# zoltanmaric/h264-fer

Measured on AMD Instinct MI355X. Metric: macroblocks/sec encode (1080p full-search ME) + bit-exact bitstream vs ref, higher is better.
Workload: dtype u8; 1 GPU; 1080p IPPP encode, full-search +-16 ME (BASELINE configs[2]); content=textured, coded_size=1920x1072, streams_per_gpu=256, contexts_per_gpu=1, gop=30, qp=12, window=32, maxdiff=3, parallelism=1 x 256 independent closed-GOP streams

## Files before the change

### h264-fer_amd/csrc/fer_me.hip

```cpp
#include <stdlib.h>
#include "fer_internal.h"
#include "fer_mvpred.h"
#include "fer_chain_idx.h"

#define INF_M 1000000000

struct WList {
    int m;
    int xy;
};

__device__ __forceinline__ int pack_xy(int x, int y) { return (x & 0xffff) | (y << 16); }
__device__ __forceinline__ int unp_x(int xy) { return (int)(short)(xy & 0xffff); }
__device__ __forceinline__ int unp_y(int xy) { return xy >> 16; }

__device__ __forceinline__ void wl_insert(WList &L, int K, int lane, bool valid, int m, int xy)
{
    int thr = lane_bcast(L.m, K - 1);
    unsigned long long mask = __ballot(valid && m < thr);
    while (mask) {
        int src = __ffsll((long long)mask) - 1;
        mask &= mask - 1;
        int cm = lane_bcast(m, src), cxy = lane_bcast(xy, src);
        int pos = __popcll(__ballot(lane < K && L.m <= cm));
        if (pos < K) {
            int um = FER_DPP(L.m, DPP_WAVE_SHR1), uxy = FER_DPP(L.xy, DPP_WAVE_SHR1);
            if (lane > pos && lane < K) {
                L.m = um;
                L.xy = uxy;
            } else if (lane == pos) {
                L.m = cm;
                L.xy = cxy;
            }
        }
    }
}

#define WAVE_LDS_SYNC()                                    \
    do {                                                   \
        __builtin_amdgcn_fence(__ATOMIC_SEQ_CST, "wavefront"); \
        __builtin_amdgcn_wave_barrier();                   \
    } while (0)
__device__ __forceinline__ int lds_rank64(const unsigned *p, unsigned mine, int n4 = 16)
{
    const uint4 *q = (const uint4 *)p;
    int r = 0;
#pragma unroll 4
    for (int i = 0; i < n4; i++) {
        uint4 k = q[i];
        r += (int)(k.x < mine) + (int)(k.y < mine) + (int)(k.z < mine) + (int)(k.w < mine);
    }
    return r;
}

template <int NB, bool ORDERED, class RAW, class FIN, class ARR>
__device__ __forceinline__ bool select_topk_ex(const int (&v)[NB], int K, int lane, int *sel, WList &L, RAW raw, FIN fin, ARR arr)
{
    unsigned *A = (unsigned *)sel, *B = A + 64;
    int *Ci = sel + 128, *Di = sel + 192;
    const unsigned long long lt = (1ull << lane) - 1ull;
    int lmin = 0x7fffffff, lmax = -1, total = 0;
#pragma unroll
    for (int u = 0; u < NB; u++) {
        total += __popcll(__ballot(v[u] >= 0));
        lmin = (int)min((unsigned)lmin, (unsigned)v[u]);
        lmax = max(lmax, v[u]);
    }
    const int need = min(K, total);
    L.m = INF_M;
    L.xy = 0;
    if (need == 0) return true;
    int c = 65;
    if (!__any(lmax >= (1 << 26))) {
        B[lane] = 0xffffffffu;
        int T0 = 0x7fffffff;
        if (__popcll(__ballot(lmin != 0x7fffffff)) >= need) {
            int lo = 0, hi = (1 << 21) - 1;
            if (__popcll(__ballot(lmin <= hi)) >= need) {
                while (lo < hi) {
                    const int mid = (lo + hi) >> 1;
                    if (__popcll(__ballot(lmin <= mid)) >= need)
                        hi = mid;
                    else
                        lo = mid + 1;
                }
                T0 = lo;
            } else {
                T0 = 1 << 21;
            }
        }
        WAVE_LDS_SYNC();
        if (T0 < (1 << 21) && NB * 64 <= 2048) {
            int nsurv = 0;
#pragma unroll
            for (int u = 0; u < NB; u++) {
                const bool take = (unsigned)v[u] <= (unsigned)T0;
                const unsigned long long mk = __ballot(take);
                if (mk) {
                    const int slot = nsurv + (int)__builtin_amdgcn_mbcnt_hi((uint32_t)(mk >> 32), __builtin_amdgcn_mbcnt_lo((uint32_t)mk, 0u));
                    if (take && slot < 64) {
                        B[slot] = ((unsigned)v[u] << 11) | (unsigned)arr(u);
                        Ci[slot] = raw(u);
                    }
                    nsurv += __popcll(mk);
                }
            }
            WAVE_LDS_SYNC();
            c = nsurv;
        }
    }
    if (c <= 64) {
        WAVE_LDS_SYNC();
        const unsigned mine = B[lane];
        const int mypay = Ci[lane];
        const int rk = lds_rank64(B, mine, (__builtin_amdgcn_readfirstlane(c) + 3) >> 2);
        WAVE_LDS_SYNC();
        if (lane < c && rk < need) {
            A[rk] = mine >> 11;
            Di[rk] = mypay;
        }
        WAVE_LDS_SYNC();
        if (lane < need) {
            L.m = (int)A[lane];
            L.xy = fin(Di[lane]);
        }
        WAVE_LDS_SYNC();
        return true;
    }
    if (!ORDERED) return false;
    int *key = sel, *kxy = sel + 64, *key2 = sel + 128, *kxy2 = sel + 192;
    int lo = wave_min(lmin), hi;
    if (__popcll(__ballot(lmin != 0x7fffffff)) >= need)
        hi = wave_max(lmin != 0x7fffffff ? lmin : -1);
    else
        hi = wave_max(lmax);
    while (lo < hi) {
        int mid = lo + ((hi - lo) >> 1);
        int cnt = 0;
#pragma unroll
        for (int u = 0; u < NB; u++) cnt += __popcll(__ballot(v[u] >= 0 && v[u] <= mid));
        if (cnt >= need)
            hi = mid;
        else
            lo = mid + 1;
    }
    const int T = lo;
    int c_less = 0;
#pragma unroll
    for (int u = 0; u < NB; u++) c_less += __popcll(__ballot(v[u] >= 0 && v[u] < T));
    const int take_eq = need - c_less;
    int nsel = 0, eq_seen = 0;
    WAVE_LDS_SYNC();
#pragma unroll
    for (int u = 0; u < NB; u++) {
        bool ok = v[u] >= 0;
        bool eq = ok && v[u] == T;
        unsigned long long meq = __ballot(eq);
        bool take = (ok && v[u] < T) || (eq && eq_seen + __popcll(meq & lt) < take_eq);
        unsigned long long mt = __ballot(take);
        if (take) {
            int pos = nsel + __popcll(mt & lt);
            key[pos] = v[u];
            kxy[pos] = raw(u);
        }
        nsel += __popcll(mt);
        eq_seen += __popcll(meq);
    }
    WAVE_LDS_SYNC();
    int mk = lane < need ? key[lane] : INF_M, mxy = lane < need ? kxy[lane] : 0;
    int rank = 0;
    for (int i = 0; i < need; i++) {
        int ki = key[i];
        rank += (ki < mk) || (ki == mk && i < lane);
    }
    if (lane < need) {
        key2[rank] = mk;
        kxy2[rank] = mxy;
    }
    WAVE_LDS_SYNC();
    if (lane < need) {
        L.m = key2[lane];
        L.xy = fin(kxy2[lane]);
    }
    WAVE_LDS_SYNC();
    return true;
}
template <int NB, class RAW, class FIN>
__device__ __forceinline__ void select_topk(const int (&v)[NB], int K, int lane, int *sel, WList &L, RAW raw, FIN fin)
{
    select_topk_ex<NB, true>(v, K, lane, sel, L, raw, fin, [&](int u) { return u * 64 + lane; });
}

typedef unsigned short u16x2_t __attribute__((ext_vector_type(2)));
typedef short i16x2_t __attribute__((ext_vector_type(2)));
__device__ __forceinline__ uint32_t pk_sub16(uint32_t a, uint32_t b)
{
    return __builtin_bit_cast(uint32_t, (u16x2_t)(__builtin_bit_cast(u16x2_t, a) - __builtin_bit_cast(u16x2_t, b)));
}
__device__ __forceinline__ uint32_t pk_abs16(uint32_t a)
{
    i16x2_t x = __builtin_bit_cast(i16x2_t, a), z = {0, 0};
    return __builtin_bit_cast(uint32_t, __builtin_elementwise_max(x, (i16x2_t)(z - x)));
}
struct SuPk {
    uint32_t s01, s23, s4;
    uint32_t d01, d23, d4;
    uint32_t s12, s34;
    uint32_t e12, e34;
};
__device__ __forceinline__ SuPk su_pack(const int s[5])
{
    SuPk p;
    p.s01 = (uint32_t)s[0] | ((uint32_t)s[1] << 16);
    p.s23 = (uint32_t)s[2] | ((uint32_t)s[3] << 16);
    p.s4 = (uint32_t)s[4];
    p.d01 = (uint32_t)(s[0] - s[1]) << 16;
    p.d23 = (uint32_t)(s[0] - s[2]) | ((uint32_t)(s[0] - s[3]) << 16);
    p.d4 = (uint32_t)(s[0] - s[4]);
    p.s12 = (uint32_t)s[1] | ((uint32_t)s[2] << 16);
    p.s34 = (uint32_t)s[3] | ((uint32_t)s[4] << 16);
    p.e12 = (uint32_t)(s[0] - s[1]) | ((uint32_t)(s[0] - s[2]) << 16);
    p.e34 = (uint32_t)(s[0] - s[3]) | ((uint32_t)(s[0] - s[4]) << 16);
    return p;
}
__device__ __forceinline__ int feat_dist_w(uint32_t a, uint32_t b, uint32_t c, const SuPk &p)
{
    uint32_t t = __builtin_amdgcn_sad_u16(a, p.s01, 0);
    t = __builtin_amdgcn_sad_u16(b, p.s23, t);
    t = __builtin_amdgcn_sad_u16(c, p.s4, t);
    uint32_t kk = __builtin_amdgcn_perm(a, a, 0x01000100);
    t = __builtin_amdgcn_sad_u16(pk_sub16(kk, a), p.d01, t);
    t = __builtin_amdgcn_sad_u16(pk_sub16(kk, b), p.d23, t);
    t = __builtin_amdgcn_sad_u16(pk_sub16(kk, c) & 0xffffu, p.d4, t);
    return (int)t;
}
__device__ __forceinline__ int feat_dist_rec(const uint16_t *__restrict__ rec, const SuPk &p)
{
    const uint32_t *r = (const uint32_t *)rec;
    return feat_dist_w(r[0], r[1], r[2], p);
}
struct FeatRec {
    uint32_t a, b, c;
};

__device__ __forceinline__ FeatRec feat_rec_direct(const IPlanes &ip, int W, int H, int frac, int refy, int refx)
{
    const int y = iclamp(refy, 0, H - 1), x = iclamp(refx, 0, W - 1);
    const uint8_t *p0 = ip.base + (size_t)frac * ip.plane + (size_t)y * ip.pitch + (x & ~3);
    const uint32_t sh = (uint32_t)(x & 3);
    uint32_t h84[8], hc[8];
#pragma unroll
    for (int r = 0; r < 8; r++) {
        const uint32_t *w = (const uint32_t *)(p0 + (size_t)r * ip.pitch);
        const uint32_t lo = __builtin_amdgcn_alignbyte(w[1], w[0], sh), hi = __builtin_amdgcn_alignbyte(w[2], w[1], sh);
        const uint32_t a4 = __builtin_amdgcn_sad_u8(lo, 0u, 0u);
        h84[r] = __builtin_amdgcn_sad_u8(hi, 0u, a4) | (a4 << 16);
        hc[r] = __builtin_amdgcn_udot4(hi, 0x00000101u, __builtin_amdgcn_udot4(lo, 0x00000101u, 0u, false), false);
    }
    const uint32_t top = h84[0] + h84[1] + h84[2] + h84[3], all = top + h84[4] + h84[5] + h84[6] + h84[7];
    const uint32_t k3 = (h84[0] + h84[1] + h84[4] + h84[5]) & 0xffffu;
    const uint32_t k4 = hc[0] + hc[1] + hc[2] + hc[3] + hc[4] + hc[5] + hc[6] + hc[7];
    FeatRec f;
    f.a = (all & 0xffffu) | (top << 16);
    f.b = (all >> 16) | (k3 << 16);
    f.c = k4;
    return f;
}

template <int R1>
struct LocalGeo {
    static constexpr int N1 = 2 * R1 + 1, PW = 2 * R1 + 8, NC = N1 * N1 * 16, NB = (NC + 63) / 64;
    static constexpr int HTAB = 8 * PW * N1 * 2;
};
template <int R1>
// ... 194 lines not shown
    const unsigned bx = xcd_swizzle(blockIdx.x, gridDim.x);
    const int mb = (int)(bx >> 2), part = (int)(bx & 3);
    const int W = d.W, H = d.H;
    const size_t ysz = d.ysz;
    const uint8_t *Y = d.curY + (size_t)s * ysz;
    const IPlanes ip = ip_stream(d, s);
    const int sx = ((mb % d.mbw) << 4) + (part & 1) * 8, sy = ((mb / d.mbw) << 4) + (part >> 1) * 8;
    const size_t pidx = ((size_t)s * d.nmb + mb) * 4 + part;

#ifdef FER_PROBE
    const bool probe = FER_DBGF(d, 128) && s == 0 && (bx % 997) == 5;
    long long tmark = probe ? wall_clock64() : 0;
#define PP_MARK(k)                                                          \
    if (probe) {                                                            \
        long long now_ = wall_clock64();                                    \
        if (lane == 0) atomicAdd((unsigned long long *)&d.timing[32 + k], (unsigned long long)(now_ - tmark)); \
        tmark = now_;                                                       \
    }
#else
#define PP_MARK(k)
#endif
    constexpr int RRL = (WIN == 16) ? 1 : 2;
    LocalLoads<RRL> ld;
    const bool fast_path = (WIN == 32 || WIN == 16) && !FER_DBGF(d, 3) && !d.basic;
    if (fast_path) local_request<RRL>(ip, W, H, sx - RRL, sy - RRL, lane, ld, 0, 1);
    int px = lane & 7, py = lane >> 3;
    int v = Y[(size_t)(sy + py) * W + sx + px];
    int su[5];
    su[0] = wave_sum(v);
    su[1] = wave_sum(py > 3 ? 0 : v);
    su[2] = wave_sum(px > 3 ? 0 : v);
    su[3] = wave_sum((py & 3) > 1 ? 0 : v);
    su[4] = wave_sum((px & 3) > 1 ? 0 : v);
    if (lane < 5) d.suma[pidx * 5 + lane] = su[lane];
    if (d.basic) {
        if (lane == 0) {
            d.st3n[pidx] = 0;
            d.v0[pidx] = 0;
        }
        return;
    }
    const SuPk sp = su_pack(su);
    PP_MARK(0)

    WList L;
    L.m = INF_M;
    L.xy = 0;
    const int R = window / 2, n = 2 * R + 1;
    const int r2 = window / 16, n2w = 2 * r2 + 1, nloc = n2w * n2w * 16;
    const uint16_t *F0 = d.feat0 + (size_t)s * 6 * ysz;
    const int wb = (n * n + 63) >> 6;
    if ((WIN == 32 || WIN == 16) && !FER_DBGF(d, 3)) {
        constexpr int WCH = 3;
        constexpr int NN = (WIN ? WIN : 32) + 1;
        constexpr int NBc = WIN ? WIN : 32, RPB = 64 / NBc, NWB = (NN + RPB - 1) / RPB;
        constexpr int LB = LocalGeo<RRL>::NB;
        static_assert(LB <= 7, "ME_SEL_NB leaves room for 7 local batches");
        const int ix = lane % NBc, r0 = lane / NBc;
        const int rx = sx - R + ix;
        const bool xok = rx >= 0 && rx < W;
        const int wx = iabs(ix - R) + 4;
        const uint32_t colo = (uint32_t)iclamp(rx, 0, W - 1) * 12u, rowb = (uint32_t)W * 12u;
        auto fin = [&](int idx) {
            if (idx < wb * 64) return pack_xy((idx / n - R) * 4, (idx % n - R) * 4);
            int c = idx - wb * 64;
            int frac = c & 15, pos = c >> 4;
            return pack_xy((pos / n2w - r2) * 4 + (frac & 3), (pos % n2w - r2) * 4 + (frac >> 2));
        };
        uint32_t k0w[NWB];
#pragma unroll
        for (int b2 = 0; b2 < NWB; b2++) {
            const int ry = iclamp(sy - R + b2 * RPB + r0, 0, H - 1);
            k0w[b2] = *(const uint32_t *)((const char *)F0 + (colo + __umul24((uint32_t)ry, rowb)));
        }
        const uint32_t k0c = feat0_load(F0, W, H, sy - R + min(lane, NN - 1), sx + R).a;
        auto second_group = [&](int half) {
            if (half == 0) local_request<RRL>(ip, W, H, sx - RRL, sy - RRL, lane, ld, 1, 2);
        };
        local_metrics<RRL, decltype(second_group), true>(ip, W, H, sx - r2, sy - r2, sp, lane, (uint32_t *)wide_m, sel_lds, 0, 2, &ld, second_group);
        unsigned lminl = 0xffffffffu;
#pragma unroll
        for (int u = 0; u < LB; u++) lminl = min(lminl, (unsigned)sel_lds[u * 64 + lane]);
        int T = 0x7fffffff;
        if (__popcll(__ballot(lminl < (1u << 21))) >= 33) {
            int lo = 0, hi = (1 << 21) - 1;
            while (lo < hi) {
                const int mid = (lo + hi) >> 1;
                if (__popcll(__ballot(lminl <= (unsigned)mid)) >= 33)
                    hi = mid;
                else
                    lo = mid + 1;
            }
            T = lo;
        }
        int *surv = wide_m;
        int ns = 0;
        const uint32_t s0 = (uint32_t)su[0];
        bool done = false;
        if (T != 0x7fffffff) {
            static_assert((NBc / 2) % RPB == 0 && NN <= 64, "a batch stays on one side of the centre row");
            const int iy_lo = max(0, R - sy), iy_hi = min(NN - 1, H - 1 - (sy - R));
            const unsigned long long rowv = ((2ull << iy_hi) - 1ull) & ~((1ull << iy_lo) - 1ull);
            const unsigned long long colv = wave_ballot(xok);
            constexpr unsigned long long GRP = NBc == 64 ? ~0ull : (1ull << NBc) - 1ull;
            const uint32_t w5lo = 5u * (uint32_t)(wx + R - r0), w5hi = 5u * (uint32_t)(wx - R + r0);
            const int arr0 = ix * NN + r0;
#pragma unroll
            for (int b2 = 0; b2 < NWB; b2++) {
                unsigned long long valid = 0;
#pragma unroll
                for (int j = 0; j < RPB; j++)
                    if ((rowv >> (b2 * RPB + j)) & 1ull) valid |= GRP << (j * NBc);
                valid &= colv;
                const uint32_t w5 = b2 * RPB < R ? w5lo - 5u * (uint32_t)(b2 * RPB) : w5hi + 5u * (uint32_t)(b2 * RPB);
                const uint32_t lb = __umul24(w5, __builtin_amdgcn_sad_u16(k0w[b2] & 0xffffu, s0, 0u));
                const unsigned long long mk = wave_ballot(lb <= (uint32_t)T) & valid;
                if (mk) {
                    const int slot = ns + (int)__builtin_amdgcn_mbcnt_hi((uint32_t)(mk >> 32), __builtin_amdgcn_mbcnt_lo((uint32_t)mk, 0u));
                    if (wave_mask_bit(mk) && slot < 128) surv[slot] = arr0 + b2 * RPB;
                    ns += __popcll(mk);
                }
            }
            {
                const uint32_t lb = __umul24(5u * (uint32_t)(R + 4 + iabs(lane - R)), __builtin_amdgcn_sad_u16(k0c & 0xffffu, s0, 0u));
                const unsigned long long mk = sx + R < W ? wave_ballot(lb <= (uint32_t)T) & rowv : 0ull;
                if (mk) {
                    const int slot = ns + (int)__builtin_amdgcn_mbcnt_hi((uint32_t)(mk >> 32), __builtin_amdgcn_mbcnt_lo((uint32_t)mk, 0u));
                    if (wave_mask_bit(mk) && slot < 128) surv[slot] = (NN - 1) * NN + lane;
                    ns += __popcll(mk);
                }
            }
            WAVE_LDS_SYNC();
            if (ns <= 128) {
                int v[2 + LB], ar[2];
#pragma unroll
                for (int b2 = 0; b2 < 2; b2++) {
                    v[b2] = -1;
                    ar[b2] = 0;
                    if (b2 * 64 < ns) {
                        const int idx = b2 * 64 + lane;
                        const bool on = idx < ns;
                        const int ai = on ? surv[idx] : 0;
                        const int cix = ai / NN, ciy = ai - cix * NN;
                        const FeatRec f = feat0_load(F0, W, H, sy - R + ciy, sx - R + cix);
                        const int m = (int)__umul24((uint32_t)(iabs(cix - R) + iabs(ciy - R) + 4), (uint32_t)feat_dist_w(f.a, f.b, f.c, sp));
                        v[b2] = on ? m : -1;
                        ar[b2] = ai;
                    }
                }
#pragma unroll
                for (int u = 0; u < LB; u++) v[2 + u] = sel_lds[u * 64 + lane];
                WAVE_LDS_SYNC();
                auto arrv = [&](int u) { return u < 2 ? ar[u < 2 ? u : 0] : wb * 64 + (u - 2) * 64 + lane; };
                done = select_topk_ex<2 + LB, false>(v, 33, lane, wide_m + 128, L, arrv, fin, arrv);
            }
        }
        PP_MARK(1)
#ifdef FER_STATS
        if (lane == 0) {
            atomicAdd((unsigned long long *)&d.timing[48], 1ull);
            atomicAdd((unsigned long long *)&d.timing[49], done ? 0ull : 1ull);
            atomicAdd((unsigned long long *)&d.timing[50], (unsigned long long)ns);
            atomicAdd((unsigned long long *)&d.timing[51], T == 0x7fffffff ? 1ull : 0ull);
            atomicAdd((unsigned long long *)&d.timing[52], (unsigned long long)(T == 0x7fffffff ? 0 : T));
        }
#endif
        if (!done) {
            WAVE_LDS_SYNC();
            int vloc[LB];
#pragma unroll
            for (int u = 0; u < LB; u++) vloc[u] = sel_lds[u * 64 + lane];
            WAVE_LDS_SYNC();
            auto wide_load = [&](int iy0, FeatRec (&fr)[WCH]) {
#pragma unroll
                for (int q = 0; q < WCH; q++) {
                    int ry = iclamp(sy - R + iy0 + q * RPB + r0, 0, H - 1);
                    const uint32_t *r = (const uint32_t *)((const char *)F0 + (colo + __umul24((uint32_t)ry, rowb)));
                    fr[q].a = r[0];
                    fr[q].b = r[1];
                    fr[q].c = r[2];
                }
            };
            auto wide_eval = [&](int iy0, const FeatRec (&fr)[WCH]) {
#pragma unroll
                for (int q = 0; q < WCH; q++) {
                    const int iy = iy0 + q * RPB + r0;
                    const int ry = sy - R + iy;
                    const int m = (int)__umul24((uint32_t)(wx + iabs(iy - R)), (uint32_t)feat_dist_w(fr[q].a, fr[q].b, fr[q].c, sp));
                    const int bad = (xok && ry >= 0 && ry < H) ? 0 : -1;
                    wide_m[iy < n ? ix * n + iy : ME_WIDE_LDS - 1] = m | bad;
                }
            };
            {
                constexpr int STEP = RPB * WCH;
                FeatRec fa[WCH], fb[WCH];
                wide_load(0, fa);
                for (int iy0 = 0; iy0 < n; iy0 += 2 * STEP) {
                    if (iy0 + STEP < n) wide_load(iy0 + STEP, fb);
                    wide_eval(iy0, fa);
                    if (iy0 + STEP < n) {
                        if (iy0 + 2 * STEP < n) wide_load(iy0 + 2 * STEP, fa);
                        wide_eval(iy0 + STEP, fb);
                    }
                }
            }
            {
                const int iy = min(lane, n - 1);
                const int rxl = sx + R, ry = sy - R + iy;
                FeatRec f = feat0_load(F0, W, H, ry, rxl);
                int m = (R + 4 + iabs(iy - R)) * feat_dist_w(f.a, f.b, f.c, sp);
                if (!(rxl < W && ry >= 0 && ry < H)) m = -1;
                if (lane < n) wide_m[(n - 1) * n + iy] = m;
            }
            __syncthreads();
            int v[ME_SEL_NB];
#pragma unroll
            for (int u = 0; u < ME_SEL_NB; u++) {
                v[u] = -1;
                if (u < wb) {
                    int c = u * 64 + lane;
                    if (c < n * n) v[u] = wide_m[c];
                } else if (u - wb < LB) {
                    v[u] = vloc[u - wb < LB ? u - wb : 0];
                }
            }
            WAVE_LDS_SYNC();
            auto raw = [&](int u) { return u * 64 + lane; };
            PP_MARK(2)
            select_topk<ME_SEL_NB>(v, 33, lane, sel_lds, L, raw, fin);
        }
        PP_MARK(3)
    } else {
        for (int base = 0; base < n * n && !FER_DBGF(d, 1); base += 64) {
            int c = base + lane;
            int tx = c / n - R, ty = c % n - R;
            int rx = sx + tx, ry = sy + ty;
            bool ok = c < n * n && rx >= 0 && rx < W && ry >= 0 && ry < H;
            int m = 0;
            if (ok) m = (iabs(tx) + iabs(ty) + 4) * feat_dist_rec(F0 + ((size_t)ry * W + rx) * 6, sp);
            wl_insert(L, 33, lane, ok, m, pack_xy(tx * 4, ty * 4));
        }
        for (int base = 0; base < nloc && !FER_DBGF(d, 2); base += 64) {
            int c = base + lane;
            int frac = c & 15, pos = c >> 4;
            int tx = pos / n2w - r2, ty = pos % n2w - r2;
            int rx = sx + tx, ry = sy + ty;
            bool ok = c < nloc && rx >= 0 && rx < W && ry >= 0 && ry < H;
            int m = 0;
            if (ok) {
                const FeatRec f = feat_rec_direct(ip, W, H, frac, ry, rx);
                m = (iabs(tx) + iabs(ty) + 4) * feat_dist_w(f.a, f.b, f.c, sp);
            }
            wl_insert(L, 33, lane, ok, m, pack_xy(tx * 4 + (frac & 3), ty * 4 + (frac >> 2)));
        }
    }
    const int n3 = __popcll(__ballot(lane < 33 && L.m < 100000000));
    int v0 = 0;
    if (!FER_DBGF(d, 4)) {
        const SrcBlk SB = src_block_load(Y, W, sx, sy);
        const int cx = unp_x(L.xy), cy = unp_y(L.xy);
        const int sad = sad_lane(ip, W, H, sx, sy, lane < n3 ? cx : 0, lane < n3 ? cy : 0, SB);
        if (lane < n3) {
            int *o = d.st3 + (pidx * 33 + lane) * 3;
            o[0] = cx;
            o[1] = cy;
            o[2] = sad;
        }
        const int wk = wave_min(lane < n3 ? (sad << 6) | lane : 0x7fffffff);
        if (wk != 0x7fffffff) v0 = lane_bcast(L.xy, wk & 63);
    }
    if (lane == 0) {
        d.st3n[pidx] = n3;
        d.v0[pidx] = v0;
    }

}

struct NoProbe {
    __device__ __forceinline__ int operator()(int) const { return 0; }
};
template <bool QUIRK, class SINK, class PROBE = NoProbe>
__device__ __forceinline__ int walk_buckets_q(const FerDev &d, int s, const int (&su)[5], const SuPk &sp, int sx, int sy, int lane,
                                              uint32_t *tbl, int halt_cnt, int &jend, SINK sink, uint32_t max_slice = 0xffffffffu,
                                              bool skip0 = false, PROBE probe = PROBE())
{
    int tren = 0;
    jend = 180;
    const int kt = d.kt;
    const uint32_t *kol2 = d.kol2 + (size_t)s * 16384 * kt;
    const uint32_t *srec = d.sort_rec;
    const int n0 = QUIRK ? d.zero_cnt[s] : 0;
    const uint32_t npos = (uint32_t)(d.W * d.H), g0 = (uint32_t)s * npos;
    const uint16_t *F0 = d.feat0 + (size_t)s * 6 * d.ysz;
    const int t_lo = QUIRK ? 0 : (max(sx - 279, 0) >> d.ktw_shift), t_hi = QUIRK ? kt - 1 : (min(sx + 279, d.W - 1) >> d.ktw_shift);
    auto qstart = [&](int a) -> uint32_t {
        if (a <= 0) return g0;
        if (a == 1) return g0 + min(2u * (uint32_t)n0, npos);
        if (a >= 16384) return g0 + npos;
        return kol2[(size_t)a * kt] - (uint32_t)n0;
    };
    const uint32_t sxy = ((uint32_t)sx << 16) | (uint32_t)sy;
    const char *srec_s = (const char *)(srec + (size_t)g0 * 3);
    auto fetch = [&](unsigned b_start, int b_cnt, uint32_t &r0, uint32_t &r1, uint32_t &r2) {
        const uint32_t li = (b_start - g0) + (unsigned)min(lane, max(b_cnt - 1, 0));
        const uint32_t *e = (const uint32_t *)(srec_s + __umul24(li, 12u));
        r0 = e[0];
        r1 = e[1];
        r2 = e[2];
    };
    auto passes = [&](uint32_t r0, uint32_t r1) -> bool {
        uint32_t dist = __builtin_amdgcn_sad_u16(r0, sxy, 0);
        uint32_t e12 = pk_abs16(pk_sub16(r1, sp.s12));
// ... 385 lines not shown
                };
                if (nout > FER_OUTL) {
                    fallback = true;
                } else {
                    const uint32_t DM = dist_of(m1, m2);
                    const bool members = halves_ok(m1);
                    bigD[q] = members && DM > 0 ? (int)DM : 0x7fffffff;
                    dminN = min(dminN, bigD[q]);
                    const uint32_t *ol = d.boutl + ((size_t)s * d.nlists + (d.kol2[((size_t)s * 16384 + bigA[q]) * d.kt] - g0_) / FER_BRANGE_MIN) * FER_OUTL;
                    for (uint32_t o0 = 0; o0 < nout; o0 += 64) {
                        const bool lv = o0 + (uint32_t)lane < nout;
                        const uint32_t idx = lv ? ol[o0 + lane] : g0_;
                        const uint32_t *rec = d.sort_rec + (size_t)idx * 3;
                        const uint32_t r0 = rec[0], r1 = rec[1], r2 = rec[2];
                        const uint32_t D = dist_of(r1, r2);
                        const bool take = lv && __builtin_amdgcn_sad_u16(r0, sxy_, 0u) < 280u && halves_ok(r1) && D > 0 && D != DM;
                        p2_add(take, (int)pk_sub16(r0, sxy_), D, jq, sideq);
                    }
                }
            }
        }
        {
            int j2, dpos = 0x7fffffff;
            walk_buckets_q<false>(d, s, su, sp, sx, sy, lane, tbl, 0x7fffffff, j2, [&](bool ok, int rank, int rel, int D, uint32_t info, bool) {
                (void)rank;
                const int j = (int)((info >> 8) & 255u);
                const bool in = j <= jend && !(j == 0 && (info >> 31));
                const bool z = in && j == 0 && ok && D == 0;
                const unsigned long long mz = __ballot(z);
                const int zr = zc + (int)__builtin_amdgcn_mbcnt_hi((uint32_t)(mz >> 32), __builtin_amdgcn_mbcnt_lo((uint32_t)mz, 0u));
                if (z && zr < 33) out[zr] = make_int2(rel, 0);
                zc += __popcll(mz);
                const bool take = in && ok && D > 0 && (j == 0 || zc < 33);
                if (take) dpos = min(dpos, D);
                p2_add(take, rel, (uint32_t)D, j, (int)(info >> 31));
                return j > jend || zc >= 33;
            }, (uint32_t)FER_BIG_SLICE, skip0);
            dmin = max(min(dmin, wave_min(dpos)), 1);
            if (zc < 33 && zc > 0) {
                __builtin_amdgcn_fence(__ATOMIC_SEQ_CST, "agent");
                const unsigned long long ev = __hip_atomic_load((const unsigned long long *)&out[min(lane, 32)], __ATOMIC_RELAXED, __HIP_MEMORY_SCOPE_AGENT);
                const int2 e = make_int2((int)(unsigned)ev, (int)(unsigned)(ev >> 32));
                if (lane < zc && zc + lane < 33) out[zc + lane] = e;
                zc = min(2 * zc, 33);
            }
        }
        if (np2 > FER_P2_CAP) fallback = true;
        if (lane == 0) {
            out[40] = make_int2(jend, dmin);
            out[41] = make_int2(min(zc, 33), (int)((uint32_t)min(np2, FER_P2_CAP) | ((uint32_t)nbig << 16) | (fallback ? 0x40000000u : 0u)));
#pragma unroll
            for (int q = 0; q < FER_BIGS; q++) out[42 + q] = make_int2(bigA[q], bigD[q]);
            out[46] = make_int2(dminN, 0);
        }
    }
    if (lane == 0) d.st2n[pidx] = tren;
}

template <int K>
__device__ __forceinline__ void sad_keys(const WList &L, int cnt, int lane, const IPlanes &ip, int W, int H, int sx, int sy,
                                         const SrcBlk &SB, int mvpx, int mvpy, int &best, int &bestxy)
{
    const bool on = lane < cnt && lane < K;
    const int cxv = on ? unp_x(L.xy) : 0, cyv = on ? unp_y(L.xy) : 0;
    const int sad = sad_lane(ip, W, H, sx, sy, cxv, cyv, SB);
    best = on ? ((sad + iabs(cxv - mvpx) + iabs(cyv - mvpy)) << 6) | lane : 0x7fffffff;
    bestxy = L.xy;
}
__device__ __forceinline__ void take_best(int best, int bestxy, int &bmin, int &bx, int &by)
{
    int wmin = wave_min(best);
    if (wmin != 0x7fffffff && (wmin >> 6) < bmin) {
        int src = __ffsll((long long)__ballot(best == wmin)) - 1;
        int xy = lane_bcast(bestxy, src);
        bmin = wmin >> 6;
        bx = unp_x(xy);
        by = unp_y(xy);
    }
}

#define ST1_UNROLL 7
#define RES_SPIN_LIMIT (1 << 23)

struct ResPre {
    int n2, n3, n2raw;
    int2 e2[FER_ST2_CAP / 64];
    int2 z;
    int c3x, c3y, c3s;
    int su[5];
    SrcBlk sb;
};

__device__ __forceinline__ void res_prefetch(const FerDev &d, int s, int gx, int gy, int lane, int role, ResPre &p)
{
    const int mb = (gy >> 1) * d.mbw + (gx >> 1), part = (gy & 1) * 2 + (gx & 1);
    const size_t pidx = ((size_t)s * d.nmb + mb) * 4 + part;
    p.n2 = p.n3 = p.n2raw = 0;
    p.z = make_int2(0, 0);
    p.c3x = p.c3y = p.c3s = 0;
#pragma unroll
    for (int u = 0; u < FER_ST2_CAP / 64; u++) p.e2[u] = make_int2(0, 0);
    if (role == 1 && !d.basic) {
        p.n2raw = d.st2n[pidx];
        p.n2 = min(p.n2raw, FER_ST2_CAP);
        p.n3 = FER_DBGF(d, 64) ? 0 : d.st3n[pidx];
        const int2 *c2 = (const int2 *)(d.st2 + pidx * FER_ST2_CAP * 2);
#pragma unroll
        for (int u = 0; u < FER_ST2_CAP / 64; u++) p.e2[u] = c2[u * 64 + lane];
        p.z = p.e2[0];
        const int *c3 = d.st3 + pidx * 33 * 3;
        const int l3 = min(lane, 32);
        p.c3x = c3[l3 * 3];
        p.c3y = c3[l3 * 3 + 1];
        p.c3s = c3[l3 * 3 + 2];
    }
#pragma unroll
    for (int k = 0; k < 5; k++) p.su[k] = d.suma[pidx * 5 + k];
    p.sb = src_block_load(d.curY + (size_t)s * d.ysz, d.W, gx * 8, gy * 8);
}

#define CH_SKIP 0x80000000u
typedef int res_i2 __attribute__((ext_vector_type(2)));
typedef int res_i3 __attribute__((ext_vector_type(3)));
typedef int res_i4 __attribute__((ext_vector_type(4)));
struct ResStage {
    res_i4 sh;
    res_i2 e1, e2;
    res_i3 c3;
    int n3;
};
__device__ __forceinline__ int res_mov(int x)
{
    int y;
    asm volatile("v_mov_b32 %0, %1" : "=v"(y) : "v"(x));
    return y;
}
struct ResNbr {
    bool vA, vB, vC, vD, vC16;
    int A, B, C, D, C16;
};

__device__ __forceinline__ void nbr_avail(int gx, int gy, int gw, bool &vB, bool &vC, bool &vD, bool &vC16)
{
    const int part = (gy & 1) * 2 + (gx & 1);
    vB = gy > 0;
    vD = gy > 0 && gx > 0;
    vC = part == 3 ? false : (part == 2 ? true : (part == 1 ? (gy > 0 && gx + 1 < gw) : gy > 0));
    vC16 = part == 0 && gy > 0 && gx + 2 < gw;
}
__device__ __forceinline__ int part_slot(int mbw, int xa, int ya) { return (((ya >> 1) * mbw + (xa >> 1)) << 2) + ((ya & 1) << 1) + (xa & 1); }

__device__ __forceinline__ void nbr_to(int v, bool ok, int &mx, int &my, int &ref)
{
    mx = ok ? (int)(short)(v & 0xffff) : FER_MV_NA;
    my = ok ? (v >> 16) : FER_MV_NA;
    ref = ok ? 0 : -1;
}
__device__ __forceinline__ void predict_nbr(bool vA, int A, bool vB, int B, bool vC, int C, bool vD, int D, int &ox, int &oy)
{
    int mx[3], my[3], ref[3];
    nbr_to(A, vA, mx[0], my[0], ref[0]);
    nbr_to(B, vB, mx[1], my[1], ref[1]);
    if (vC)
        nbr_to(C, true, mx[2], my[2], ref[2]);
    else
        nbr_to(D, vD, mx[2], my[2], ref[2]);
    predict_core(mx, my, ref, ox, oy);
}

__device__ __forceinline__ void wave_best(int best, int bestxy, int &wkey, int &wxy)
{
    wkey = wave_min(best);
    wxy = 0;
    if (wkey != 0x7fffffff) wxy = lane_bcast(bestxy, __ffsll((long long)__ballot(best == wkey)) - 1);
}

__device__ __forceinline__ void pskip_vector(const FerDev &d, int mb, int mbx, const ResNbr &N, int &smx, int &smy)
{
    smx = smy = 0;
    if (!(mb < d.mbw || mbx == 0)) {
        const bool zu = N.B == 0, zl = N.A == 0;
        if (!(zu || zl)) predict_nbr(N.vA, N.A, N.vB, N.B, N.vC16, N.C16, N.vD, N.D, smx, smy);
    }
}
__device__ __forceinline__ bool pskip_test(const FerDev &d, int s, int mbx, int mby, int lane, int smx, int smy)
{
    const int W = d.W, H = d.H;
    const uint8_t *Y = d.curY + (size_t)s * d.ysz;
    const uint8_t *RY = d.refY + (size_t)s * d.ysz;
    const IPlanes ip = ip_stream(d, s);
    const int xp = mbx << 4, yp = mby << 4;
    const int lx = (lane & 3) * 4, ly = lane >> 2;
    int srcv[4], pred[4];
    const uint32_t sv = *(const uint32_t *)(Y + (size_t)(yp + ly) * W + xp + lx);
#pragma unroll
    for (int k = 0; k < 4; k++) srcv[k] = (sv >> (8 * k)) & 0xff;
    mc_luma4(RY, ip, W, H, xp, yp, lx, ly, smx, smy, pred);
    int MAXDIFF = d.maxdiff_set;
    if (d.maxdiff_set == -1) {
        int mean = wave_sum(srcv[0] + srcv[1] + srcv[2] + srcv[3]) / 256;
        int dev = wave_sum(iabs(srcv[0] - mean) + iabs(srcv[1] - mean) + iabs(srcv[2] - mean) + iabs(srcv[3] - mean));
        MAXDIFF = dev / 256;
        if (MAXDIFF < 3) MAXDIFF = 3;
    }
    bool exact = true;
#pragma unroll
    for (int k = 0; k < 4; k++) exact = exact && iabs(srcv[k] - pred[k]) <= MAXDIFF;
    return __all(exact);
}

template <int WIN>
__device__ __forceinline__ int stage1_list(const FerDev &d, int s, int gx, int gy, int lane, const ResPre &P, int genx, int geny,
                                           int *sel_lds, const int *mtab, WList &L1)
{
    const int window = WIN ? WIN : d.window;
    const int W = d.W, H = d.H;
    const int sx = gx * 8, sy = gy * 8;
    L1.m = INF_M;
    L1.xy = 0;
    if (FER_DBGF(d, 16)) return 0;
    const int r1 = window / 16, n1 = 2 * r1 + 1, tot1 = n1 * n1 * 16;
    auto raw1 = [&](int u) { return u * 64 + lane; };
    auto fin1 = [&](int cc) {
        int frac = cc & 15, pos = cc >> 4;
        return pack_xy((genx - r1 + pos / n1) * 4 + (frac & 3), (geny - r1 + pos % n1) * 4 + (frac >> 2));
    };
    if (WIN == 32 || WIN == 16) {
        constexpr int RR = (WIN ? WIN : 32) / 16;
        constexpr int NB1 = LocalGeo<RR>::NB;
        int m[NB1];
#pragma unroll
        for (int u = 0; u < NB1; u++) m[u] = mtab[u * 64 + lane];
        select_topk<NB1>(m, 17, lane, sel_lds, L1, raw1, fin1);
    } else {
        const SuPk sp = su_pack(P.su);
        const IPlanes ip = ip_stream(d, s);
        for (int base = 0; base < tot1; base += 64) {
            int cc = base + lane;
            int frac = cc & 15, pos = cc >> 4;
            int tx = genx - r1 + pos / n1, ty = geny - r1 + pos % n1;
            int rx = sx + tx, ry = sy + ty;
            bool ok = cc < tot1 && rx >= 0 && rx < W && ry >= 0 && ry < H;
            int m = 0;
            if (ok) {
                const FeatRec f = feat_rec_direct(ip, W, H, frac, ry, rx);
                m = (iabs(tx - genx) + iabs(ty - geny) + 4) * feat_dist_w(f.a, f.b, f.c, sp);
            }
            wl_insert(L1, 17, lane, ok, m, pack_xy(tx * 4 + (frac & 3), ty * 4 + (frac >> 2)));
        }
    }
    return __popcll(__ballot(lane < 17 && L1.m < 100000000));
}

template <int WIN>
__device__ __forceinline__ void resolve_stage1(const FerDev &d, int s, int gx, int gy, int lane, const ResPre &P, int mvpx, int mvpy,
                                               uint32_t *htab, int *mtab, int &wkey, int &wxy)
{
    wkey = 0x7fffffff;
    wxy = 0;
    if (FER_DBGF(d, 16)) return;
    if (WIN == 32 || WIN == 16) {
        constexpr int RR = (WIN ? WIN : 32) / 16;
        local_metrics<RR>(ip_stream(d, s), d.W, d.H, gx * 8 + (mvpx >> 2) - RR, gy * 8 + (mvpy >> 2) - RR, su_pack(P.su), lane, htab, mtab);
    }
    WList L1;
    const int cnt1 = stage1_list<WIN>(d, s, gx, gy, lane, P, mvpx >> 2, mvpy >> 2, (int *)htab, mtab, L1);
    if (FER_DBGF(d, 16)) return;
    int b1, b1xy;
    sad_keys<17>(L1, cnt1, lane, ip_stream(d, s), d.W, d.H, gx * 8, gy * 8, P.sb, mvpx, mvpy, b1, b1xy);
    wave_best(b1, b1xy, wkey, wxy);
}

struct CList {
    int m;
    unsigned ak;
    int xy;
};
__device__ __forceinline__ void cl_insert(CList &L, int lane, bool valid, int m, unsigned ak, int xy)
{
    const int tm = lane_bcast(L.m, 32);
    const unsigned tk = (unsigned)lane_bcast((int)L.ak, 32);
    unsigned long long mask = __ballot(valid && (m < tm || (m == tm && ak < tk)));
    while (mask) {
        const int src = __ffsll((long long)mask) - 1;
        mask &= mask - 1;
        const int cm = lane_bcast(m, src), cxy = lane_bcast(xy, src);
        const unsigned ck = (unsigned)lane_bcast((int)ak, src);
        const int pos = __popcll(__ballot(lane < 33 && (L.m < cm || (L.m == cm && L.ak < ck))));
        if (pos < 33) {
            const int um = FER_DPP(L.m, DPP_WAVE_SHR1), uxy = FER_DPP(L.xy, DPP_WAVE_SHR1);
            const unsigned uk = (unsigned)FER_DPP((int)L.ak, DPP_WAVE_SHR1);
            if (lane > pos && lane < 33) {
                L.m = um;
                L.ak = uk;
                L.xy = uxy;
            } else if (lane == pos) {
                L.m = cm;
                L.ak = ck;
                L.xy = cxy;
            }
        }
    }
}

__device__ __forceinline__ void resolve_crowded(const FerDev &d, int s, int sx, int sy, int lane, const ResPre &P, int genx, int geny,
                                                WList &L2)
{
    const int W = d.W, H = d.H;
    const uint16_t *F0 = d.feat0 + (size_t)s * 6 * d.ysz;
    const SuPk sp = su_pack(P.su);
    const int J = lane_bcast(P.e2[0].x, 40), zc = lane_bcast(P.e2[0].x, 41);
    const uint32_t fl = (uint32_t)lane_bcast(P.e2[0].y, 41);
    const bool classes = (fl & 0x40000000u) == 0;
    const int np2 = classes ? (int)(fl & 0xffffu) : 0, nbig = classes ? (int)((fl >> 16) & 15u) : 0;
    const int dmin = classes ? lane_bcast(P.e2[0].x, 46) : lane_bcast(P.e2[0].y, 40);
    int bigA[FER_BIGS], bigD[FER_BIGS];
#pragma unroll
    for (int q = 0; q < FER_BIGS; q++) {
        bigA[q] = lane_bcast(P.e2[0].x, 42 + q);
        bigD[q] = lane_bcast(P.e2[0].y, 42 + q);
    }
    CList L;
    L.m = INF_M;
    L.ak = 0xffffffffu;
    L.xy = 0;
    if (lane < zc) {
        const int rel = P.z.x;
        const int tx = rel >> 16, ty = (int)(short)(rel & 0xffff);
        L.m = 0;
        L.ak = (unsigned)lane;
        L.xy = pack_xy(tx * 4, ty * 4);
    }
    if (zc < 33) {
#pragma unroll
        for (int u = 1; u < FER_ST2_CAP / 64; u++) {
            if ((u - 1) * 64 < np2) {
                const bool on = (u - 1) * 64 + lane < np2;
                const int rel = P.e2[u].x;
                const uint32_t pk = (uint32_t)P.e2[u].y;
                const int tx = rel >> 16, ty = (int)(short)(rel & 0xffff);
                const int D = (int)(pk & 0xfffffu), j = (int)((pk >> 20) & 255u);
                const unsigned side = (pk >> 28) & 1u;
                const int m = (iabs(tx - genx) + iabs(ty - geny) + 4) * D;
                const unsigned akey = ((unsigned)j << 21) | ((unsigned)(tx + 280) << 10) | (unsigned)(ty + 280);
                const int xy = pack_xy(tx * 4, ty * 4);
                cl_insert(L, lane, on, m, akey | (side << 20), xy);
                if (__any(on && j == 0)) cl_insert(L, lane, on && j == 0, m, akey | (1u << 20), xy);
            }
        }
    }
    if (zc < 33 && dmin != 0x7fffffff) {
        const int cx = sx + genx, cy = sy + geny;
        const int rmax = 2 * 280 + iabs(genx) + iabs(geny);
        int done_r = -1;
        for (int k0 = 0;; k0 += 64) {
            const int k = k0 + lane;
            int r = 0, i = 0;
            if (k > 0) {
                r = (int)((1.0f + __fsqrt_rn((float)(2 * k - 1))) * 0.5f);
                while (2 * r * (r - 1) + 1 > k) r--;
                while (2 * (r + 1) * r + 1 <= k) r++;
                i = k - (2 * r * (r - 1) + 1);
            }
            int dx = 0, dy = 0;
            if (r > 0) {
                const int q = i / r, t = i - q * r;
                dx = q == 0 ? r - t : (q == 1 ? -t : (q == 2 ? t - r : t));
                dy = q == 0 ? t : (q == 1 ? r - t : (q == 2 ? -t : t - r));
            }
            const int px = cx + dx, py = cy + dy;
            const bool inpic = px >= 0 && px < W && py >= 0 && py < H;
            const uint32_t *rec = (const uint32_t *)((const char *)F0 + (__umul24((uint32_t)iclamp(py, 0, H - 1), (uint32_t)W * 12u) + (uint32_t)iclamp(px, 0, W - 1) * 12u));
            const uint32_t a = rec[0], b = rec[1], c = rec[2];
            const int kk0 = (int)(a & 0xffffu), kk1 = (int)(a >> 16), kk2 = (int)(b & 0xffffu);
            const int j = iabs(kk0 - P.su[0]);
            const int tx = px - sx, ty = py - sy;
            const bool member = inpic && j <= J && iabs(tx) + iabs(ty) < 280 && iabs(kk1 - P.su[1]) < 100 && iabs(kk2 - P.su[2]) < 100;
            const int D = feat_dist_w(a, b, c, sp);
            bool take = member && D > 0;
            if (classes) {
                bool cls = false;
#pragma unroll
                for (int q = 0; q < FER_BIGS; q++) cls = cls || (q < nbig && kk0 == bigA[q] && D == bigD[q]);
                take = take && cls;
            }
            const int m = (r + 4) * D;
            const int side = kk0 > P.su[0] ? 1 : 0;
            const unsigned akey = ((unsigned)j << 21) | ((unsigned)(tx + 280) << 10) | (unsigned)(ty + 280);
            const int xy = pack_xy(tx * 4, ty * 4);
            cl_insert(L, lane, take, m, akey | ((unsigned)side << 20), xy);
            if (__any(take && j == 0)) cl_insert(L, lane, take && j == 0, m, akey | (1u << 20), xy);
            {
                int rr = (int)((1.0f + __fsqrt_rn((float)(2 * (k0 + 64) - 1))) * 0.5f);
                while (2 * rr * (rr - 1) + 1 > k0 + 64) rr--;
                while (2 * (rr + 1) * rr + 1 <= k0 + 64) rr++;
                done_r = rr - 1;
            }
            const int t33 = lane_bcast(L.m, 32);
            if (done_r >= rmax) break;
            if (t33 < INF_M && (long long)(done_r + 1 + 4) * dmin > (long long)t33) break;
        }
    }
    L2.m = L.m;
    L2.xy = L.xy;
}

__device__ __forceinline__ int stage2_list(const FerDev &d, int s, int gx, int gy, int lane, const ResPre &P, int genx, int geny,
                                           int *sel_lds, WList &L2)
{
    const int sx = gx * 8, sy = gy * 8;
    L2.m = INF_M;
    L2.xy = 0;
    if (d.basic || FER_DBGF(d, 32)) return 0;
    const uint32_t cfl = (uint32_t)lane_bcast(P.e2[0].y, 41);
    const bool rewalk = (cfl & 0x40000000u) != 0 && ((cfl >> 16) & 15u) == 0;
    if (P.n2raw > FER_ST2_CAP && d.zero_cnt[s] == 0 && !rewalk) {
        resolve_crowded(d, s, sx, sy, lane, P, genx, geny, L2);
    } else if (P.n2raw > FER_ST2_CAP) {
        const SuPk sp = su_pack(P.su);
        int jx;
        walk_buckets(d, s, P.su, sp, sx, sy, lane, (uint32_t *)sel_lds, 0x7fffffff, jx, [&](bool ok, int rank, int rel, int D, uint32_t, bool) {
            (void)rank;
            int tx = rel >> 16, ty = (int)(short)(rel & 0xffff);
            wl_insert(L2, 33, lane, ok, (iabs(tx - genx) + iabs(ty - geny) + 4) * D, pack_xy(tx * 4, ty * 4));
            return false;
        });
    } else {
        int m2[FER_ST2_CAP / 64];
#pragma unroll
        for (int u = 0; u < FER_ST2_CAP / 64; u++) {
            int cc = u * 64 + lane;
            int tx = P.e2[u].x >> 16, ty = (int)(short)(P.e2[u].x & 0xffff);
            m2[u] = (int)__umul24((uint32_t)(iabs(tx - genx) + iabs(ty - geny) + 4), (uint32_t)P.e2[u].y) | (cc < P.n2 ? 0 : -1);
        }
        auto raw2 = [&](int u) { return P.e2[u].x; };
        auto fin2 = [&](int e) { return pack_xy((e >> 16) * 4, (int)(short)(e & 0xffff) * 4); };
        select_topk<FER_ST2_CAP / 64>(m2, 33, lane, sel_lds, L2, raw2, fin2);
    }
    return __popcll(__ballot(lane < 33 && L2.m < 100000000));
}

template <int WIN>
__device__ __forceinline__ void resolve_stage23(const FerDev &d, int s, int gx, int gy, int lane, const ResPre &P, int mvpx, int mvpy,
                                                int *sel_lds, int &k2, int &xy2, int &k3, int &xy3)
{
    k2 = k3 = 0x7fffffff;
    xy2 = xy3 = 0;
    if (d.basic || FER_DBGF(d, 32)) return;
    WList L2;
    const int cnt2 = stage2_list(d, s, gx, gy, lane, P, mvpx >> 2, mvpy >> 2, sel_lds, L2);
    if (FER_DBGF(d, 256)) L2.xy = pack_xy(lane & 7, lane >> 3);
    int b2, b2xy;
    sad_keys<33>(L2, cnt2, lane, ip_stream(d, s), d.W, d.H, gx * 8, gy * 8, P.sb, mvpx, mvpy, b2, b2xy);
    wave_best(b2, b2xy, k2, xy2);
    int key = 0x7fffffff;
    if (lane < P.n3) key = ((P.c3s + iabs(P.c3x - mvpx) + iabs(P.c3y - mvpy)) << 6) | lane;
    wave_best(key, pack_xy(P.c3x, P.c3y), k3, xy3);
}

__device__ __forceinline__ ResNbr nbr_from_field(const FerDev &d, const int *vf, int gx, int gy, int lane)
{
    ResNbr N;
    nbr_avail(gx, gy, d.mbw * 2, N.vB, N.vC, N.vD, N.vC16);
    N.vA = gx > 0;
    const int xa = gx + (lane == 0 ? 0 : (lane == 1 ? 1 : (lane == 2 ? -1 : (lane == 3 ? 2 : -1)))), ya = lane == 4 ? gy : gy - 1;
    const bool val = lane == 0 ? N.vB : (lane == 1 ? N.vC : (lane == 2 ? N.vD : (lane == 3 ? N.vC16 : (lane == 4 && N.vA))));
    const int w = val ? vf[part_slot(d.mbw, xa, ya)] : 0;
    N.B = lane_bcast(w, 0);
    N.C = lane_bcast(w, 1);
    N.D = lane_bcast(w, 2);
    N.C16 = lane_bcast(w, 3);
    N.A = lane_bcast(w, 4);
    return N;
}

#ifndef SPEC_WAVES
#define SPEC_WAVES 7
#endif
template <int WIN>
__global__ __launch_bounds__(256) __attribute__((amdgpu_waves_per_eu(SPEC_WAVES, SPEC_WAVES))) void k_me_spec(FerDev d)
{
    __shared__ __attribute__((aligned(16))) uint32_t loc_all[4][LocalGeo<2>::HTAB + LocalGeo<2>::NB * 64];
    __shared__ int skipflag;
    static_assert(LocalGeo<2>::HTAB >= 256, "the selection's scratch fits the row sums");
    const int lane = threadIdx.x & 63;
    const int part = __builtin_amdgcn_readfirstlane(threadIdx.x >> 6);
    const int s = blockIdx.y;
    if (d.hdr[s * 4 + 3] != 0) return;
    const int mb = (int)xcd_swizzle(blockIdx.x, gridDim.x);
    const int mbx = mb % d.mbw, mby = mb / d.mbw;
    const int gx = mbx * 2 + (part & 1), gy = mby * 2 + (part >> 1);
    const size_t pidx = ((size_t)s * d.nmb + mb) * 4 + part;
    uint32_t *htab = loc_all[part];
    int *mtab = (int *)loc_all[part] + LocalGeo<2>::HTAB;
    int *sel_lds = (int *)loc_all[part];
    const ResNbr N = nbr_from_field(d, d.v0 + (size_t)s * d.nmb * 4, gx, gy, lane);
    int mvpx, mvpy;
    predict_nbr(N.vA, N.A, N.vB, N.B, N.vC, N.C, N.vD, N.D, mvpx, mvpy);
    const int genx = mvpx >> 2, geny = mvpy >> 2;
    const int genw = pack_xy(genx, geny);
    const int W = d.W, H = d.H;
    const IPlanes ip = ip_stream(d, s);
    const int sx = gx * 8, sy = gy * 8;
    constexpr int RRL = (WIN == 16) ? 1 : 2;
    LocalLoads<RRL> ld;
    if (WIN == 32 || WIN == 16) local_request<RRL>(ip, W, H, sx + genx - RRL, sy + geny - RRL, lane, ld);
    ResPre P;
    res_prefetch(d, s, gx, gy, lane, 1, P);
    int smw = 0;
    bool sk = false;
    if (part == 0) {
        int smx, smy;
        pskip_vector(d, mb, mbx, N, smx, smy);
        smw = pack_xy(smx, smy);
        sk = pskip_test(d, s, mbx, mby, lane, smx, smy);
        if (lane == 0) skipflag = sk;
    }
    __syncthreads();
    sk = skipflag != 0;
    if (sk) {
// ... 359 lines not shown
```

Before: 23.28 million macroblocks/s.

## Coarsen top-k threshold search, use scalar ballot counts, split stage-2 list loads

```diff
diff --git a/h264-fer_amd/csrc/fer_me.hip b/h264-fer_amd/csrc/fer_me.hip
--- a/h264-fer_amd/csrc/fer_me.hip
+++ b/h264-fer_amd/csrc/fer_me.hip
@@ -1,7 +1,9 @@
 #include <stdlib.h>
+#include <type_traits>
 #include "fer_internal.h"
 #include "fer_mvpred.h"
 #include "fer_chain_idx.h"
+#include "fer_sel_thr.h"
 
 #define INF_M 1000000000
 
@@ -53,8 +55,23 @@
     return r;
 }
 
-template <int NB, bool ORDERED, class RAW, class FIN, class ARR>
-__device__ __forceinline__ bool select_topk_ex(const int (&v)[NB], int K, int lane, int *sel, WList &L, RAW raw, FIN fin, ARR arr)
+__device__ __forceinline__ int wave_count(bool p)
+{
+    int n;
+    asm("s_bcnt1_i32_b64 %0, %1" : "=s"(n) : "s"(__builtin_amdgcn_ballot_w64(p)) : "scc");
+    return n;
+}
+#ifdef FER_STATS
+#define SEL_STAT(k)                                                                        \
+    do {                                                                                   \
+        if (stat && lane == 0) atomicAdd((unsigned long long *)&stat[k], 1ull);            \
+    } while (0)
+#else
+#define SEL_STAT(k) (void)stat
+#endif
+
+template <int NB, bool ORDERED, bool COARSE, class RAW, class FIN, class ARR>
+__device__ __forceinline__ bool select_topk_ex(const int (&v)[NB], int K, int lane, int *sel, WList &L, RAW raw, FIN fin, ARR arr, long long *stat = nullptr)
 {
     unsigned *A = (unsigned *)sel, *B = A + 64;
     int *Ci = sel + 128, *Di = sel + 192;
@@ -62,7 +79,7 @@
     int lmin = 0x7fffffff, lmax = -1, total = 0;
 #pragma unroll
     for (int u = 0; u < NB; u++) {
-        total += __popcll(__ballot(v[u] >= 0));
+        total += wave_count(v[u] >= 0);
         lmin = (int)min((unsigned)lmin, (unsigned)v[u]);
         lmax = max(lmax, v[u]);
     }
@@ -70,45 +87,52 @@
     L.m = INF_M;
     L.xy = 0;
     if (need == 0) return true;
+    SEL_STAT(0);
     int c = 65;
     if (!__any(lmax >= (1 << 26))) {
-        B[lane] = 0xffffffffu;
         int T0 = 0x7fffffff;
-        if (__popcll(__ballot(lmin != 0x7fffffff)) >= need) {
-            int lo = 0, hi = (1 << 21) - 1;
-            if (__popcll(__ballot(lmin <= hi)) >= need) {
-                while (lo < hi) {
-                    const int mid = (lo + hi) >> 1;
-                    if (__popcll(__ballot(lmin <= mid)) >= need)
-                        hi = mid;
-                    else
-                        lo = mid + 1;
-                }
-                T0 = lo;
+        bool exact = true;
+        if (wave_count(lmin != 0x7fffffff) >= need) {
+            if (wave_count(lmin <= FER_SEL_LIMIT - 1) >= need) {
+                if (COARSE) {
+                    const int lcode = sel_code_of((unsigned)lmin);
+                    T0 = sel_thr(sel_search_bits<FER_SEL_CODE_BITS, FER_SEL_CODE_BITS>(need, [&](int trial) { return wave_count(lcode < trial); }));
+                    exact = false;
+                } else {
+                    T0 = sel_search_bits<21, 1>(need, [&](int trial) { return wave_count(lmin < trial); });
+                }
             } else {
-                T0 = 1 << 21;
-            }
-        }
-        WAVE_LDS_SYNC();
-        if (T0 < (1 << 21) && NB * 64 <= 2048) {
-            int nsurv = 0;
-#pragma unroll
-            for (int u = 0; u < NB; u++) {
-                const bool take = (unsigned)v[u] <= (unsigned)T0;
-                const unsigned long long mk = __ballot(take);
-                if (mk) {
-                    const int slot = nsurv + (int)__builtin_amdgcn_mbcnt_hi((uint32_t)(mk >> 32), __builtin_amdgcn_mbcnt_lo((uint32_t)mk, 0u));
-                    if (take && slot < 64) {
-                        B[slot] = ((unsigned)v[u] << 11) | (unsigned)arr(u);
-                        Ci[slot] = raw(u);
+                T0 = FER_SEL_LIMIT;
+            }
+        }
+        if (T0 < FER_SEL_LIMIT && NB * 64 <= 2048) {
+            for (;;) {
+                B[lane] = 0xffffffffu;
+                WAVE_LDS_SYNC();
+                int nsurv = 0;
+#pragma unroll
+                for (int u = 0; u < NB; u++) {
+                    const bool take = (unsigned)v[u] <= (unsigned)T0;
+                    const unsigned long long mk = __ballot(take);
+                    if (mk) {
+                        const int slot = nsurv + (int)__builtin_amdgcn_mbcnt_hi((uint32_t)(mk >> 32), __builtin_amdgcn_mbcnt_lo((uint32_t)mk, 0u));
+                        if (take && slot < 64) {
+                            B[slot] = ((unsigned)v[u] << 11) | (unsigned)arr(u);
+                            Ci[slot] = raw(u);
+                        }
+                        nsurv += (int)__builtin_popcountll(mk);
                     }
-                    nsurv += __popcll(mk);
-                }
-            }
-            WAVE_LDS_SYNC();
-            c = nsurv;
-        }
-    }
+                }
+                WAVE_LDS_SYNC();
+                c = nsurv;
+                if (c <= 64 || exact) break;
+                SEL_STAT(1);
+                T0 = sel_search_bits<21, 1>(need, [&](int trial) { return wave_count(lmin < trial); });
+                exact = true;
+            }
+        }
+    }
+    if (c > 64) SEL_STAT(2);
     if (c <= 64) {
         WAVE_LDS_SYNC();
         const unsigned mine = B[lane];
@@ -185,11 +209,16 @@
     WAVE_LDS_SYNC();
     return true;
 }
-template <int NB, class RAW, class FIN>
-__device__ __forceinline__ void select_topk(const int (&v)[NB], int K, int lane, int *sel, WList &L, RAW raw, FIN fin)
-{
-    select_topk_ex<NB, true>(v, K, lane, sel, L, raw, fin, [&](int u) { return u * 64 + lane; });
-}
+template <int NB, bool COARSE = true, class RAW, class FIN>
+__device__ __forceinline__ void select_topk(const int (&v)[NB], int K, int lane, int *sel, WList &L, RAW raw, FIN fin, long long *stat = nullptr)
+{
+    select_topk_ex<NB, true, COARSE>(v, K, lane, sel, L, raw, fin, [&](int u) { return u * 64 + lane; }, stat);
+}
+#define SEL_SITE_ST1 8
+#define SEL_SITE_ST2 11
+#define SEL_SITE_ST3 14
+#define SEL_SITE_ST3_FULL 17
+#define SEL_SITE_N2_HI 20
 
 typedef unsigned short u16x2_t __attribute__((ext_vector_type(2)));
 typedef short i16x2_t __attribute__((ext_vector_type(2)));
@@ -550,16 +579,8 @@
 #pragma unroll
         for (int u = 0; u < LB; u++) lminl = min(lminl, (unsigned)sel_lds[u * 64 + lane]);
         int T = 0x7fffffff;
-        if (__popcll(__ballot(lminl < (1u << 21))) >= 33) {
-            int lo = 0, hi = (1 << 21) - 1;
-            while (lo < hi) {
-                const int mid = (lo + hi) >> 1;
-                if (__popcll(__ballot(lminl <= (unsigned)mid)) >= 33)
-                    hi = mid;
-                else
-                    lo = mid + 1;
-            }
-            T = lo;
+        if (wave_count(lminl < (1u << 21)) >= 33) {
+            T = sel_search_bits<21, 21>(33, [&](int trial) { return wave_count(lminl < (unsigned)trial); });
         }
         int *surv = wide_m;
         int ns = 0;
@@ -620,7 +641,7 @@
                 for (int u = 0; u < LB; u++) v[2 + u] = sel_lds[u * 64 + lane];
                 WAVE_LDS_SYNC();
                 auto arrv = [&](int u) { return u < 2 ? ar[u < 2 ? u : 0] : wb * 64 + (u - 2) * 64 + lane; };
-                done = select_topk_ex<2 + LB, false>(v, 33, lane, wide_m + 128, L, arrv, fin, arrv);
+                done = select_topk_ex<2 + LB, false, true>(v, 33, lane, wide_m + 128, L, arrv, fin, arrv, d.timing + SEL_SITE_ST3);
             }
         }
         PP_MARK(1)
@@ -695,7 +716,7 @@
             WAVE_LDS_SYNC();
             auto raw = [&](int u) { return u * 64 + lane; };
             PP_MARK(2)
-            select_topk<ME_SEL_NB>(v, 33, lane, sel_lds, L, raw, fin);
+            select_topk<ME_SEL_NB, false>(v, 33, lane, sel_lds, L, raw, fin, d.timing + SEL_SITE_ST3_FULL);
         }
         PP_MARK(3)
     } else {
@@ -1247,9 +1268,11 @@
 #define ST1_UNROLL 7
 #define RES_SPIN_LIMIT (1 << 23)
 
+#define ST2_NB (FER_ST2_CAP / 64)
+#define ST2_NB_LO (ST2_NB / 2)
 struct ResPre {
     int n2, n3, n2raw;
-    int2 e2[FER_ST2_CAP / 64];
+    int2 e2[ST2_NB];
     int2 z;
     int c3x, c3y, c3s;
     int su[5];
@@ -1271,7 +1294,7 @@
         p.n3 = FER_DBGF(d, 64) ? 0 : d.st3n[pidx];
         const int2 *c2 = (const int2 *)(d.st2 + pidx * FER_ST2_CAP * 2);
 #pragma unroll
-        for (int u = 0; u < FER_ST2_CAP / 64; u++) p.e2[u] = c2[u * 64 + lane];
+        for (int u = 0; u < ST2_NB_LO; u++) p.e2[u] = c2[u * 64 + lane];
         p.z = p.e2[0];
         const int *c3 = d.st3 + pidx * 33 * 3;
         const int l3 = min(lane, 32);
@@ -1282,6 +1305,11 @@
 #pragma unroll
     for (int k = 0; k < 5; k++) p.su[k] = d.suma[pidx * 5 + k];
     p.sb = src_block_load(d.curY + (size_t)s * d.ysz, d.W, gx * 8, gy * 8);
+    if (role == 1 && !d.basic && __builtin_amdgcn_readfirstlane(p.n2raw) > ST2_NB_LO * 64) {
+        const int2 *c2 = (const int2 *)(d.st2 + pidx * FER_ST2_CAP * 2);
+#pragma unroll
+        for (int u = ST2_NB_LO; u < ST2_NB; u++) p.e2[u] = c2[u * 64 + lane];
+    }
 }
 
 #define CH_SKIP 0x80000000u
@@ -1396,7 +1424,7 @@
         int m[NB1];
 #pragma unroll
         for (int u = 0; u < NB1; u++) m[u] = mtab[u * 64 + lane];
-        select_topk<NB1>(m, 17, lane, sel_lds, L1, raw1, fin1);
+        select_topk<NB1>(m, 17, lane, sel_lds, L1, raw1, fin1, d.timing + SEL_SITE_ST1);
     } else {
         const SuPk sp = su_pack(P.su);
         const IPlanes ip = ip_stream(d, s);
@@ -1498,7 +1526,7 @@
     }
     if (zc < 33) {
 #pragma unroll
-        for (int u = 1; u < FER_ST2_CAP / 64; u++) {
+        for (int u = 1; u < ST2_NB; u++) {
             if ((u - 1) * 64 < np2) {
                 const bool on = (u - 1) * 64 + lane < np2;
                 const int rel = P.e2[u].x;
@@ -1591,16 +1619,26 @@
             return false;
         });
     } else {
-        int m2[FER_ST2_CAP / 64];
-#pragma unroll
-        for (int u = 0; u < FER_ST2_CAP / 64; u++) {
-            int cc = u * 64 + lane;
-            int tx = P.e2[u].x >> 16, ty = (int)(short)(P.e2[u].x & 0xffff);
-            m2[u] = (int)__umul24((uint32_t)(iabs(tx - genx) + iabs(ty - geny) + 4), (uint32_t)P.e2[u].y) | (cc < P.n2 ? 0 : -1);
-        }
         auto raw2 = [&](int u) { return P.e2[u].x; };
         auto fin2 = [&](int e) { return pack_xy((e >> 16) * 4, (int)(short)(e & 0xffff) * 4); };
-        select_topk<FER_ST2_CAP / 64>(m2, 33, lane, sel_lds, L2, raw2, fin2);
+        auto over = [&](auto nb) {
+            constexpr int NB = decltype(nb)::value;
+            int m2[NB];
+#pragma unroll
+            for (int u = 0; u < NB; u++) {
+                int cc = u * 64 + lane;
+                int tx = P.e2[u].x >> 16, ty = (int)(short)(P.e2[u].x & 0xffff);
+                m2[u] = (int)__umul24((uint32_t)(iabs(tx - genx) + iabs(ty - geny) + 4), (uint32_t)P.e2[u].y) | (cc < P.n2 ? 0 : -1);
+            }
+            select_topk<NB>(m2, 33, lane, sel_lds, L2, raw2, fin2, d.timing + SEL_SITE_ST2);
+        };
+#ifdef FER_STATS
+        if (lane == 0 && P.n2 > ST2_NB_LO * 64) atomicAdd((unsigned long long *)&d.timing[SEL_SITE_N2_HI], 1ull);
+#endif
+        if (__builtin_amdgcn_readfirstlane(P.n2) <= ST2_NB_LO * 64)
+            over(std::integral_constant<int, ST2_NB_LO>());
+        else
+            over(std::integral_constant<int, ST2_NB>());
     }
     return __popcll(__ballot(lane < 33 && L2.m < 100000000));
 }
diff --git a/h264-fer_amd/csrc/fer_sel_thr.h b/h264-fer_amd/csrc/fer_sel_thr.h
--- /dev/null
+++ b/h264-fer_amd/csrc/fer_sel_thr.h
@@ -0,0 +1,38 @@
+#pragma once
+
+#ifdef __HIPCC__
+#define FER_SEL_HD __host__ __device__ inline
+#else
+#define FER_SEL_HD inline
+#endif
+
+#define FER_SEL_LIMIT (1 << 21)
+#define FER_SEL_CODE_MAX 151
+#define FER_SEL_CODE_BITS 8
+
+FER_SEL_HD int sel_code_of(unsigned t)
+{
+    if (t < 8u) return (int)t;
+    const int e = 31 - __builtin_clz(t);
+    return ((e - 2) << 3) | (int)((t >> (e - 3)) & 7u);
+}
+
+FER_SEL_HD int sel_thr(int code)
+{
+    const int E = code >> 3, mant = code & 7;
+    if (E == 0) return mant;
+    if (E > 18) return FER_SEL_LIMIT - 1;
+    return ((9 + mant) << (E - 1)) - 1;
+}
+
+template <int BITS, int UNROLL, class COUNT>
+FER_SEL_HD int sel_search_bits(int need, COUNT count_below)
+{
+    int r = 0;
+#pragma unroll UNROLL
+    for (int b = BITS - 1; b >= 0; b--) {
+        const int trial = r | (1 << b);
+        r = count_below(trial) < need ? trial : r;
+    }
+    return r;
+}
```

New measurement: 24.12 million macroblocks/s, median of 6. +3.6%, better.
